# EnyaHermite/SPH3D-GCN

Measured on AMD Instinct MI355X. Metric: point-cloud blocks/sec (fwd+bwd) SPH3D_s3dis 8192-pt, higher is better.
Workload: dtype f32

## Files before the change

### sph3d_gcn_amd/csrc/conv3d.hip

```cpp
#include <stddef.h>
#include <string.h>
#include <type_traits>
#include "common.hpp"
#include "conv_plan.hpp"

namespace sph3d {

constexpr int kFwdSB = 4;
constexpr int kBatch = 8;

template <int R, int LPE, int SB>
__global__ __launch_bounds__(64 * kMultiWaves) void dwconv_fwd_multi(
    int B, int N, int M, int F, int C, int K, int mblocks, int nslices,
    const int* __restrict__ nnIndex, const int* __restrict__ nnCount, const int* __restrict__ binIndex,
    const float* __restrict__ input, const float* __restrict__ filter, float* __restrict__ output)
{
    extern __shared__ __attribute__((aligned(16))) float lfilt[];
    constexpr int EPL = 64 / LPE;
    constexpr int NO = 4 * R;
    constexpr int SLI = 4 * LPE;
    constexpr int FSTB = SLI * R * 4;
    const int CR = C * R;
    int b, part;
    xcd_decode((int)blockIdx.x, B, mblocks * nslices, b, part);
    if (b < 0) return;
    const int slice = part / mblocks;
    const int mb = part - slice * mblocks;
    const int ci0 = slice * SLI;
    const int SLi = (C - ci0) < SLI ? (C - ci0) : SLI;
    const int SLo = SLi * R;

    for (int e = threadIdx.x * 4; e < F * SLo; e += blockDim.x * 4) {
        const int f = e / SLo;
        const int cl = e - f * SLo;
        const int l4 = cl / (4 * R), q = (cl >> 2) % R;
        *reinterpret_cast<float4*>(&lfilt[f * (SLI * R) + q * SLI + l4 * 4]) =
            *reinterpret_cast<const float4*>(&filter[(size_t)f * CR + ci0 * R + cl]);
    }
    for (int e = threadIdx.x; e < SLI * R; e += blockDim.x) lfilt[F * (SLI * R) + e] = 0.f;
    __syncthreads();

    const int wave = uniform((int)threadIdx.x >> 6);
    const int lane = lane_id();
    const int g = lane / LPE;
    const int li = lane - g * LPE;
    const bool act = li * 4 < SLi;
    const int cic = act ? li * 4 : 0;
    const int m_begin = mb * kMultiPoints;
    const int m_end = (m_begin + kMultiPoints) < M ? (m_begin + kMultiPoints) : M;
    const char* inb = reinterpret_cast<const char*>(input + (size_t)b * N * C + ci0);
    const unsigned cicb = (unsigned)cic * 4u;
    const unsigned rowb = (unsigned)C * 4u;
    const char* lfb = reinterpret_cast<const char*>(lfilt);

    for (int m = m_begin + wave; m < m_end; m += kMultiWaves) {
        const size_t row = (size_t)b * M + m;
        const int cnt = uniform(nnCount[row]);
        float acc[NO];
#pragma unroll
        for (int v = 0; v < NO; v++) acc[v] = 0.f;
        for (int kt = 0; kt < cnt; kt += 64) {
            const int myk = kt + lane;
            const int kn = (cnt - kt) < 64 ? (cnt - kt) : 64;
            const int mykc = myk < cnt ? myk : kt;
            const int idxv = nnIndex[row * K + mykc];
            int binv = binIndex[row * K + mykc];
            binv = binv < 0 ? 0 : (binv >= F ? F - 1 : binv);
            binv = myk < cnt ? binv : F;
            const unsigned pk = ((unsigned)idxv & 0xffffffu) | ((unsigned)binv << 24);
            static_assert(64 % (SB * EPL) == 0, "batches must tile the 64-edge chunk (no index clamps)");
            for (int k0 = 0; k0 < kn; k0 += SB * EPL) {
                float4 x[SB];
                unsigned fo[SB];
#pragma unroll
                for (int u = 0; u < SB; u++) {
                    const int kq = k0 + u * EPL + g;
                    const unsigned p = (unsigned)__shfl((int)pk, kq);
                    const unsigned off = __umul24(p, rowb) + cicb;
                    fo[u] = __umul24(p >> 24, (unsigned)FSTB) + cicb;
                    x[u] = *reinterpret_cast<const float4*>(inb + off);
                }
#pragma unroll
                for (int u = 0; u < SB; u++) {
                    const float xs[4] = {x[u].x, x[u].y, x[u].z, x[u].w};
#pragma unroll
                    for (int q = 0; q < R; q++) {
                        const float4 w = *reinterpret_cast<const float4*>(lfb + fo[u] + q * (SLI * 4));
                        acc[4 * q + 0] = fmaf(xs[(4 * q + 0) / R], w.x, acc[4 * q + 0]);
                        acc[4 * q + 1] = fmaf(xs[(4 * q + 1) / R], w.y, acc[4 * q + 1]);
                        acc[4 * q + 2] = fmaf(xs[(4 * q + 2) / R], w.z, acc[4 * q + 2]);
                        acc[4 * q + 3] = fmaf(xs[(4 * q + 3) / R], w.w, acc[4 * q + 3]);
                    }
                }
            }
        }
#pragma unroll
        for (int o = LPE; o < 64; o <<= 1)
#pragma unroll
            for (int v = 0; v < NO; v++) acc[v] += __shfl_xor(acc[v], o);
        if (act && g == 0) {
            const float inv = cnt > 0 ? 1.0f / (float)cnt : 0.f;
            float* op = &output[row * CR + (size_t)(ci0 + li * 4) * R];
#pragma unroll
            for (int q = 0; q < R; q++) {
                float4 o;
                o.x = acc[4 * q + 0] * inv;
                o.y = acc[4 * q + 1] * inv;
                o.z = acc[4 * q + 2] * inv;
                o.w = acc[4 * q + 3] * inv;
                *reinterpret_cast<float4*>(&op[4 * q]) = o;
            }
        }
    }
}

template <int R>
__global__ __launch_bounds__(256) void dwconv_fwd_row(
    int B, int N, int M, int F, int C, int K, int mblocks, int nslices,
    const int* __restrict__ nnIndex, const int* __restrict__ nnCount, const int* __restrict__ binIndex,
    const float* __restrict__ input, const float* __restrict__ filter, float* __restrict__ output,
    const float* __restrict__ input2 = nullptr, int Ca = 0)
{
    extern __shared__ __attribute__((aligned(16))) float lfilt[];
    const int CR = C * R;
    int b, part;
    xcd_decode((int)blockIdx.x, B, mblocks * nslices, b, part);
    if (b < 0) return;
    const int slice = part / mblocks;
    const int mb = part - slice * mblocks;
    const int slice0 = slice * kSlice;
    const int SL = (CR - slice0) < kSlice ? (CR - slice0) : kSlice;

    for (int e = threadIdx.x * 4; e < F * SL; e += blockDim.x * 4) {
        const int f = e / SL;
        const int cl = e - f * SL;
        *reinterpret_cast<float4*>(&lfilt[e]) = *reinterpret_cast<const float4*>(&filter[(size_t)f * CR + slice0 + cl]);
    }
    for (int e = threadIdx.x; e < SL; e += blockDim.x) lfilt[F * SL + e] = 0.f;
    __syncthreads();

    const int wave = uniform((int)threadIdx.x >> 6);
    const int lane = lane_id();
    const int cl0 = lane * 4;
    const bool act = cl0 < SL;
    const int cin0 = (slice0 + cl0) / R;
    const int clc = act ? cl0 : 0;
    const int cinc = act ? cin0 : slice0 / R;
    const int m_begin = mb * kFwdPointsPerWG;
    const int m_end = (m_begin + kFwdPointsPerWG) < M ? (m_begin + kFwdPointsPerWG) : M;
    const bool second = input2 != nullptr && (slice0 / R) >= Ca;
    const int Cs = input2 == nullptr ? C : (second ? C - Ca : Ca);
    const int cshift = second ? Ca : 0;
    const float* inb = (second ? input2 : input) + (size_t)b * N * Cs - cshift;

    for (int m = m_begin + wave; m < m_end; m += 4) {
        const size_t row = (size_t)b * M + m;
        const int cnt = uniform(nnCount[row]);
        float4 acc = make_float4(0.f, 0.f, 0.f, 0.f);
        for (int kt = 0; kt < cnt; kt += 64) {
            const int myk = kt + lane;
            const int kn = (cnt - kt) < 64 ? (cnt - kt) : 64;
            const int mykc = myk < cnt ? myk : kt;
            const int idxv = nnIndex[row * K + mykc];
            int binv = binIndex[row * K + mykc];
            binv = binv < 0 ? 0 : (binv >= F ? F - 1 : binv);
            binv = myk < cnt ? binv : F;
            const unsigned noff = (unsigned)idxv * (unsigned)Cs;
            const int foff = binv * (SL >> 2);
            for (int k8 = 0; k8 < kn; k8 += kBatch) {
                unsigned n[kBatch];
                int f[kBatch];
#pragma unroll
                for (int u = 0; u < kBatch; u++) {
                    n[u] = (unsigned)__builtin_amdgcn_readlane((int)noff, k8 + u);
                    f[u] = __builtin_amdgcn_readlane(foff, k8 + u);
                }
                float4 w[kBatch];
                float4 x[kBatch];
#pragma unroll
                for (int u = 0; u < kBatch; u++) {
                    w[u] = reinterpret_cast<const float4*>(lfilt)[f[u] + (clc >> 2)];
                    const float* __restrict__ rp = inb + n[u];
                    if (R == 2) {
                        const float2 t = *reinterpret_cast<const float2*>(&rp[(unsigned)cinc]);
                        x[u] = make_float4(t.x, t.x, t.y, t.y);
                    } else {
                        x[u] = *reinterpret_cast<const float4*>(&rp[(unsigned)cinc]);
                    }
                }
#pragma unroll
                for (int u = 0; u < kBatch; u++) {
                    acc.x = fmaf(x[u].x, w[u].x, acc.x);
                    acc.y = fmaf(x[u].y, w[u].y, acc.y);
                    acc.z = fmaf(x[u].z, w[u].z, acc.z);
                    acc.w = fmaf(x[u].w, w[u].w, acc.w);
                }
            }
        }
        if (act) {
            const float inv = cnt > 0 ? 1.0f / (float)cnt : 0.f;
            float4 o;
            o.x = acc.x * inv;
            o.y = acc.y * inv;
            o.z = acc.z * inv;
            o.w = acc.w * inv;
            *reinterpret_cast<float4*>(&output[row * CR + slice0 + cl0]) = o;
        }
    }
}

__global__ __launch_bounds__(256) void dwconv_fwd_generic(
    int B, int N, int M, int F, int C, int r, int K, int mblocks, int nslices,
    const int* __restrict__ nnIndex, const int* __restrict__ nnCount, const int* __restrict__ binIndex,
    const float* __restrict__ input, const float* __restrict__ filter, float* __restrict__ output)
{
    extern __shared__ __attribute__((aligned(16))) float lfilt[];
    const int CR = C * r;
    int b, part;
    xcd_decode((int)blockIdx.x, B, mblocks * nslices, b, part);
    if (b < 0) return;
    const int slice = part / mblocks;
    const int mb = part - slice * mblocks;
    const int slice0 = slice * kSlice;
    const int SL = (CR - slice0) < kSlice ? (CR - slice0) : kSlice;

    for (int e = threadIdx.x; e < F * SL; e += blockDim.x) {
        const int f = e / SL;
        const int cl = e - f * SL;
        lfilt[e] = filter[(size_t)f * CR + slice0 + cl];
    }
    __syncthreads();

    const int wave = uniform((int)threadIdx.x >> 6);
    const int lane = lane_id();
    int cl[4], cin[4];
    bool act[4];
#pragma unroll
    for (int t = 0; t < 4; t++) {
        cl[t] = lane + 64 * t;
        act[t] = cl[t] < SL;
        cin[t] = act[t] ? (slice0 + cl[t]) / r : 0;
        if (!act[t]) cl[t] = 0;
    }
    const int m_begin = mb * kFwdPointsPerWG;
    const int m_end = (m_begin + kFwdPointsPerWG) < M ? (m_begin + kFwdPointsPerWG) : M;
    const float* inb = input + (size_t)b * N * C;

    for (int m = m_begin + wave; m < m_end; m += 4) {
        const size_t row = (size_t)b * M + m;
        const int cnt = uniform(nnCount[row]);
        float acc[4] = {0.f, 0.f, 0.f, 0.f};
        const int* __restrict__ irow = nnIndex + row * K;
        const int* __restrict__ brow = binIndex + row * K;
        {
#pragma unroll 4
            for (int kk = 0; kk < cnt; kk++) {
                const int n = irow[kk];
                int f = brow[kk];
                f = f < 0 ? 0 : (f >= F ? F - 1 : f);
#pragma unroll
                for (int t = 0; t < 4; t++) {
                    const float x = inb[(size_t)n * C + cin[t]];
                    const float w = lfilt[f * SL + cl[t]];
                    acc[t] = fmaf(x, w, acc[t]);
                }
            }
        }
#pragma unroll
        for (int t = 0; t < 4; t++) {
            if (act[t]) output[row * CR + slice0 + cl[t]] = cnt > 0 ? acc[t] / (float)cnt : 0.f;
        }
    }
}


constexpr int kBwdNL2 = 3;
constexpr int kBwdNL4 = 2;
template <int R, int V, int MAXF, int PARTS, bool COMPACT, int HUB = 0>
__global__ __launch_bounds__(kBwdTWaves * 64, COMPACT ? 4 : 3) void dwconv_bwd_t_vec(
    int B, int N, int M, int F, int C, int W, int parts, int nslices,
    const int* __restrict__ offsets, const int* __restrict__ entKey, const float* __restrict__ entScale,
    const int* __restrict__ order, const int* __restrict__ activeBins, int compactMax,
    const float* __restrict__ input, const float* __restrict__ filter, const float* __restrict__ gradOutput,
    float* __restrict__ gradInput, float* __restrict__ partial,
    const float* __restrict__ input2 = nullptr, float* __restrict__ gradInput2 = nullptr, int Ca = 0,
    int* __restrict__ hubList = nullptr, int hubT = 0, int slabBase = 0)
{
    extern __shared__ __attribute__((aligned(16))) float lds[];
    constexpr int SLW = 64 * V;
    constexpr int VI = (V >= R) ? V / R : 1;
    const int CR = C * R;
    const int A = activeBins ? uniform(activeBins[0]) : F;
    if (COMPACT ? (A > MAXF) : (activeBins != nullptr && A <= compactMax)) return;
    const int xcd = HUB == 2 ? 0 : ((int)blockIdx.x & 7);
    const int q = HUB == 2 ? (int)blockIdx.x : ((int)blockIdx.x >> 3);
    const int slice = q / W;
    const int w = q - slice * W;
    const int slice0 = slice * SLW;
    const int SL = (CR - slice0) < SLW ? (CR - slice0) : SLW;
    float* lfilt = lds;
    const bool second = input2 != nullptr && (slice0 / R) >= Ca;
    const int Cs = input2 == nullptr ? C : (second ? C - Ca : Ca);
    const float* __restrict__ xin = (second ? input2 : input) - (second ? Ca : 0);
    float* __restrict__ gin = (second ? gradInput2 : gradInput) - (second ? Ca : 0);

    for (int e = threadIdx.x * V; e < F * SL; e += blockDim.x * V) {
        const int f = e / SL;
        const int cl = e - f * SL;
#pragma unroll
        for (int v = 0; v < V; v++) lfilt[e + v] = filter[(size_t)f * CR + slice0 + cl + v];
    }
    __syncthreads();

    const int wave = uniform((int)threadIdx.x >> 6);
    const int lane = lane_id();
    const int stride = W * kBwdTWaves;
    constexpr bool HALF = PARTS > 1;
    constexpr int PL = 64 / PARTS;
    const int half = HALF ? (lane / PL) : 0;
    const int cl0 = (HALF ? (lane % PL) : lane) * V;
    const bool act = cl0 < SL;
    const int cin0 = (slice0 + cl0) / R;
    float acc[MAXF][V];
#pragma unroll
    for (int i = 0; i < MAXF; i++)
#pragma unroll
        for (int v = 0; v < V; v++) acc[i][v] = 0.f;

    const int abv = COMPACT ? activeBins[1 + ((lane < MAXF && lane < A) ? lane : 0)] : 0;

    const int nhub = HUB == 2 ? uniform(hubList[0]) : 0;
    for (int item = HUB == 2 ? w / kHubGroup : xcd; HUB == 2 ? item < nhub : item < B * parts; item += HUB == 2 ? W / kHubGroup : 8) {
    const int hubSrc = HUB == 2 ? uniform(hubList[1 + item]) : 0;
    const int b = HUB == 2 ? hubSrc / N : item / parts;
    const int pi = HUB == 2 ? 0 : item - b * parts;
    const float* __restrict__ gou = gradOutput + (size_t)b * M * CR + slice0;
    const unsigned cla = (unsigned)(act ? cl0 : 0);
    const int* __restrict__ offb = offsets + (size_t)b * ((size_t)N * F + 1);
    for (int p = HUB == 2 ? 0 : pi + parts * (w * kBwdTWaves + wave); HUB == 2 ? p < 1 : p < N; p += HUB == 2 ? 1 : parts * stride) {
        const int n = HUB == 2 ? hubSrc - b * N : (order ? uniform(order[(size_t)b * N + p]) : p);
        const int* __restrict__ o = offb + (size_t)n * F;
        const int ov0 = o[lane <= F ? lane : F];
        const int ov1 = (MAXF >= 64) ? o[(64 + lane) <= F ? (64 + lane) : F] : 0;
        float xi[VI], xv[V];
#pragma unroll
        for (int u = 0; u < VI; u++) xi[u] = xin[((size_t)b * N + n) * Cs + (act ? cin0 : slice0 / R) + u];
#pragma unroll
        for (int v = 0; v < V; v++) xv[v] = xi[(V >= R) ? v / R : 0];
        float gi[V];
#pragma unroll
        for (int v = 0; v < V; v++) gi[v] = 0.f;
        const int E0 = __builtin_amdgcn_readlane(ov0, 0);
        const int E1 = uniform(o[F]);
        unsigned long long nonempty = ~0ull;
        if (COMPACT) {
            const int fl = lane < MAXF ? abv : 0;
            const int s0 = __builtin_amdgcn_ds_bpermute(fl << 2, ov0);
            const int s1 = __builtin_amdgcn_ds_bpermute((fl + 1) << 2, ov0);
            nonempty = __ballot(s1 > s0);
        }
        if (HUB == 1 && (E1 - E0) > hubT) {
            if (slice == 0 && lane == 0) hubList[1 + atomicAdd(&hubList[0], 1)] = b * N + n;
            if (act && half == 0 && V >= R) {
                float* gp = &gin[((size_t)b * N + n) * Cs + cin0];
#pragma unroll
                for (int u = 0; u < VI; u++) gp[u] = 0.f;
            }
            continue;
        }
        const int cfirst = HUB == 2 ? E0 + 64 * ((w % kHubGroup) * kBwdTWaves + wave) : E0;
        const int cstep = HUB == 2 ? 64 * kHubGroup * kBwdTWaves : 64;
        for (int cb = cfirst; cb < E1; cb += cstep) {
        const int cn = (E1 - cb) < 64 ? (E1 - cb) : 64;
        const int li = lane < cn ? lane : 0;
        const int wkey = entKey[cb + li];
        const unsigned kel = (unsigned)tg_key(wkey, entScale == nullptr) * (unsigned)CR;
        const float svl = entScale == nullptr ? tg_packed_scale(wkey) : entScale[cb + li];
        const float sv = lane < cn ? svl : 0.f;
#pragma unroll
        for (int fi = 0; fi < MAXF; fi++) {
            if (fi < (COMPACT ? A : F) && (!COMPACT || ((nonempty >> (fi & 63)) & 1ull))) {
                const int f = COMPACT ? __builtin_amdgcn_readlane(abv, fi) : fi;
                const int a0 = COMPACT ? __builtin_amdgcn_readlane(ov0, f)
                                       : __builtin_amdgcn_readlane(fi < 64 ? ov0 : ov1, fi & 63);
                const int a1 = COMPACT ? __builtin_amdgcn_readlane(ov0, f + 1)
                                       : __builtin_amdgcn_readlane((fi + 1) < 64 ? ov0 : ov1, (fi + 1) & 63);
                const int e0 = (a0 > cb ? a0 : cb) - cb;
                const int e1 = (a1 < cb + cn ? a1 : cb + cn) - cb;
                if (e0 < e1) {
                    float sg[V];
#pragma unroll
                    for (int v = 0; v < V; v++) sg[v] = 0.f;
                    float wr[V];
                    {
                        const float* wrow = &lfilt[f * SL + (act ? cl0 : 0)];
#pragma unroll
                        for (int v = 0; v < V; v++) wr[v] = wrow[v];
                    }
                    if (HALF) {
                        constexpr int NL = PARTS == 2 ? kBwdNL2 : kBwdNL4;
                        const float svh = ((unsigned)(lane - e0) < (unsigned)(e1 - e0)) ? sv : 0.f;
#define SPH3D_BWD_HALF_BATCH(WRAPS)                                                                                  \
    {                                                                                                                \
        const int a4 = ((e + half) << 2);                                                                            \
        unsigned ko[NL];                                                                                             \
        float sc[NL];                                                                                                \
        _Pragma("unroll") for (int u = 0; u < NL; u++) {                                                             \
            ko[u] = (unsigned)__builtin_amdgcn_ds_bpermute(a4 + 4 * PARTS * u, (int)kel);                            \
            sc[u] = __int_as_float(__builtin_amdgcn_ds_bpermute(a4 + 4 * PARTS * u, __float_as_int(svh)));           \
            if (WRAPS) sc[u] = (e + half + PARTS * u) < 64 ? sc[u] : 0.f;                                            \
        }                                                                                                            \
        float g[NL][V];                                                                                              \
        _Pragma("unroll") for (int u = 0; u < NL; u++) {                                                             \
            const float4 t = *reinterpret_cast<const float4*>(&gou[ko[u] + cla]);                                    \
            g[u][0] = t.x; g[u][1 % V] = t.y; g[u][2 % V] = t.z; g[u][3 % V] = t.w;                                  \
        }                                                                                                            \
        _Pragma("unroll") for (int u = 0; u < NL; u++)                                                               \
            _Pragma("unroll") for (int v = 0; v < V; v++) sg[v] = fmaf(g[u][v], sc[u], sg[v]);                       \
    }
                        for (int e = e0; e < e1; e += PARTS * NL) {
                            if ((64 % (PARTS * NL)) != 0 && e + PARTS * NL > 64) SPH3D_BWD_HALF_BATCH(true)
                            else SPH3D_BWD_HALF_BATCH(false)
                        }
#undef SPH3D_BWD_HALF_BATCH
                    } else {
                    const float svm = ((unsigned)(lane - e0) < (unsigned)(e1 - e0)) ? sv : 0.f;
#define SPH3D_BWD_BATCH(NB)                                                                                          \
    {                                                                                                                \
        float sc[NB];                                                                                                \
        float g[NB][V];                                                                                              \
        _Pragma("unroll") for (int u = 0; u < NB; u++) {                                                             \
            const unsigned ko = (unsigned)__builtin_amdgcn_readlane((int)kel, e + u);                                \
            sc[u] = __int_as_float(__builtin_amdgcn_readlane(__float_as_int(svm), e + u));                           \
            const float* __restrict__ rp = gou + ko;                                   \
                        \
            if (V == 4) {                                                                                            \
                const float4 t = *reinterpret_cast<const float4*>(&rp[cla]);                                         \
                g[u][0] = t.x; g[u][1 % V] = t.y; g[u][2 % V] = t.z; g[u][3 % V] = t.w;                              \
            } else if (V == 2) {                                                                                     \
                const float2 t = *reinterpret_cast<const float2*>(&rp[cla]);                                         \
                g[u][0] = t.x; g[u][1 % V] = t.y;                                                                    \
            } else {                                                                                                 \
                g[u][0] = rp[cla];                                                                                   \
            }                                                                                                        \
        }                                                                                                            \
        _Pragma("unroll") for (int u = 0; u < NB; u++)                                                               \
            _Pragma("unroll") for (int v = 0; v < V; v++) sg[v] = fmaf(g[u][v], sc[u], sg[v]);                       \
    }
                    int e = e0;
                    for (; e + 4 <= e1; e += 4) SPH3D_BWD_BATCH(4)
                    const int rem = e1 - e;
                    if (rem == 3) SPH3D_BWD_BATCH(3)
                    else if (rem == 2) SPH3D_BWD_BATCH(2)
                    else if (rem == 1) SPH3D_BWD_BATCH(1)
#undef SPH3D_BWD_BATCH
                    }
#pragma unroll
                    for (int v = 0; v < V; v++) {
                        gi[v] = fmaf(sg[v], wr[v], gi[v]);
                        acc[fi][v] = fmaf(sg[v], xv[v], acc[fi][v]);
                    }
                }
            }
        }
        }
        if (HALF) {
#pragma unroll
            for (int v = 0; v < V; v++) {
                gi[v] += __shfl_xor(gi[v], 32);
                if (PARTS == 4) gi[v] += __shfl_xor(gi[v], 16);
            }
        }
        if (act && half == 0) {
            float* gp = &gin[((size_t)b * N + n) * Cs + cin0];
            if (V >= R) {
#pragma unroll
                for (int u = 0; u < VI; u++) {
                    float s = 0.f;
#pragma unroll
                    for (int rr = 0; rr < R; rr++) s += gi[u * R + rr];
                    if (HUB == 2) atomicAdd(&gp[u], s);
                    else gp[u] = s;
                }
            }
        }
    }

    }

    if (HALF) {
#pragma unroll
        for (int i = 0; i < MAXF; i++)
#pragma unroll
            for (int v = 0; v < V; v++) {
                acc[i][v] += __shfl_xor(acc[i][v], 32);
                if (PARTS == 4) acc[i][v] += __shfl_xor(acc[i][v], 16);
            }
    }
    __syncthreads();
    float* tab = lds;
    __shared__ unsigned long long activeMask;
    if (COMPACT) {
        if (threadIdx.x == 0) activeMask = 0ull;
        __syncthreads();
        if ((int)threadIdx.x < A) atomicOr(&activeMask, 1ull << activeBins[1 + threadIdx.x]);
        __syncthreads();
    }
    for (int w = 0; w < kBwdTWaves; w++) {
        if (wave == w && act && half == 0) {
#pragma unroll
            for (int i = 0; i < MAXF; i++) {
                if (i < (COMPACT ? A : F)) {
                    const int f = COMPACT ? uniform(activeBins[1 + i]) : i;
#pragma unroll
                    for (int v = 0; v < V; v++) {
                        float* p = &tab[f * SL + cl0 + v];
                        *p = (w == 0) ? acc[i][v] : (*p + acc[i][v]);
                    }
                }
            }
        }
        __syncthreads();
    }
    float* out = partial + (HUB == 2 ? (size_t)slabBase + w : (size_t)xcd * W + w) * ((size_t)F * CR);
    const unsigned long long am = COMPACT ? activeMask : ~0ull;
    for (int e = threadIdx.x; e < F * SL; e += blockDim.x) {
        const int f = e / SL;
        const int cl = e - f * SL;
        if (!COMPACT || ((am >> f) & 1ull)) out[(size_t)f * CR + slice0 + cl] = tab[e];
    }
}

__global__ __launch_bounds__(1024) void reduce_filter_partials(int nparts, int total, int CR, const float* __restrict__ partial,
                                                              float* __restrict__ gradFilter,
                                                              const int* __restrict__ activeBins, int compactMax, int npartsCompact)
{
    const bool compact = activeBins != nullptr && activeBins[0] <= compactMax;
    if (compact) nparts = npartsCompact;
    __shared__ float red[32][32];
    __shared__ unsigned long long activeMask;
    if (compact) {
        if (threadIdx.x == 0) activeMask = 0ull;
        __syncthreads();
        if ((int)threadIdx.x < activeBins[0]) atomicOr(&activeMask, 1ull << activeBins[1 + threadIdx.x]);
        __syncthreads();
    }
    const int cx = (int)threadIdx.x & 31, py = (int)threadIdx.x >> 5;
    const int j = blockIdx.x * 32 + cx;
    float s = 0.f;
    if (j < total && (!compact || ((activeMask >> (j / CR)) & 1ull))) {
        for (int p0 = py; p0 < nparts; p0 += 256) {
            float v[8];
#pragma unroll
            for (int u = 0; u < 8; u++) {
                const int p = p0 + u * 32;
                v[u] = partial[(size_t)(p < nparts ? p : py) * total + j];
            }
#pragma unroll
            for (int u = 0; u < 8; u++)
                if (p0 + u * 32 < nparts) s += v[u];
        }
    }
    red[py][cx] = s;
    __syncthreads();
    if (py == 0 && j < total) {
        for (int k = 1; k < 32; k++) s += red[k][cx];
        gradFilter[j] = s;
    }
}

__global__ __launch_bounds__(256) void dwconv_bwd_t_generic(
    int B, int N, int M, int F, int C, int r, int nblocks, int nslices, int sliceC,
    const int* __restrict__ offsets, const int* __restrict__ entKey, const float* __restrict__ entScale,
    const float* __restrict__ input, const float* __restrict__ filter, const float* __restrict__ gradOutput,
    float* __restrict__ gradInput, float* __restrict__ gradFilter)
{
    extern __shared__ __attribute__((aligned(16))) float gtab[];
    const int CR = C * r;
    int b, part;
    xcd_decode((int)blockIdx.x, B, nblocks * nslices, b, part);
    if (b < 0) return;
    const int slice = part / nblocks;
    const int nb = part - slice * nblocks;
    const int c_base = slice * sliceC;
    const int SC = (C - c_base) < sliceC ? (C - c_base) : sliceC;
    const int SW = SC * r;
    for (int e = threadIdx.x; e < F * SW; e += blockDim.x) gtab[e] = 0.f;
    __syncthreads();

    const int wave = uniform((int)threadIdx.x >> 6);
    const int lane = lane_id();
    const int n_begin = nb * 64;
    const int n_end = (n_begin + 64) < N ? (n_begin + 64) : N;
    const int* __restrict__ offb = offsets + (size_t)b * ((size_t)N * F + 1);
    for (int n = n_begin + wave; n < n_end; n += 4) {
        const int* __restrict__ o = offb + (size_t)n * F;
        for (int t = 0; t < 4; t++) {
            const int cl = lane + 64 * t;
            if (cl >= SC) break;
            const int cin = c_base + cl;
            const float x = input[((size_t)b * N + n) * C + cin];
            float gi = 0.f;
            for (int f = 0; f < F; f++) {
                const int e0 = o[f], e1 = o[f + 1];
                if (e0 >= e1) continue;
                for (int rr = 0; rr < r; rr++) {
                    const int cout = cin * r + rr;
                    float sg = 0.f;
                    for (int e = e0; e < e1; e++)
                        sg = fmaf(gradOutput[((size_t)b * M + tg_key(entKey[e], entScale == nullptr)) * CR + cout],
                                  entScale == nullptr ? tg_packed_scale(entKey[e]) : entScale[e], sg);
                    gi = fmaf(sg, filter[(size_t)f * CR + cout], gi);
                    unsafeAtomicAdd(&gtab[f * SW + cl * r + rr], sg * x);
                }
            }
            gradInput[((size_t)b * N + n) * C + cin] = gi;
        }
    }
    __syncthreads();
    for (int e = threadIdx.x; e < F * SW; e += blockDim.x) {
        const int f = e / SW;
        const int j = e - f * SW;
        const float g = gtab[e];
        if (g != 0.f) unsafeAtomicAdd(&gradFilter[(size_t)f * CR + c_base * r + j], g);
    }
}

template <int T, int MAXF>
__global__ __launch_bounds__(kBwdTWaves * 64, 3) void dwconv_bwd_t_odd(
    int B, int N, int M, int F, int C, int W, int parts, int nslices,
    const int* __restrict__ offsets, const int* __restrict__ entKey, const float* __restrict__ entScale,
    const int* __restrict__ order,
    const float* __restrict__ input, const float* __restrict__ filter, const float* __restrict__ gradOutput,
    float* __restrict__ gradInput, float* __restrict__ partial)
{
    extern __shared__ __attribute__((aligned(16))) float lds[];
    constexpr int SLW = 64 * T;
    const int xcd = (int)blockIdx.x & 7;
    const int q = (int)blockIdx.x >> 3;
    const int slice = q / W;
    const int w = q - slice * W;
    const int slice0 = slice * SLW;
    const int SL = (C - slice0) < SLW ? (C - slice0) : SLW;
    float* lfilt = lds;
    for (int e = threadIdx.x; e < F * SLW; e += blockDim.x) {
        const int f = e / SLW;
        const int cl = e - f * SLW;
        lfilt[e] = cl < SL ? filter[(size_t)f * C + slice0 + cl] : 0.f;
    }
    __syncthreads();

    const int wave = uniform((int)threadIdx.x >> 6);
    const int lane = lane_id();
    const int stride = W * kBwdTWaves;
    bool act[T];
    unsigned cla[T];
#pragma unroll
    for (int t = 0; t < T; t++) {
        act[t] = lane + 64 * t < SL;
        cla[t] = act[t] ? (unsigned)(lane + 64 * t) : 0u;
    }
    float acc[MAXF][T];
#pragma unroll
    for (int i = 0; i < MAXF; i++)
#pragma unroll
        for (int t = 0; t < T; t++) acc[i][t] = 0.f;

    for (int item = xcd; item < B * parts; item += 8) {
    const int b = item / parts;
    const int pi = item - b * parts;
    const float* __restrict__ gou = gradOutput + (size_t)b * M * C + slice0;
    const int* __restrict__ offb = offsets + (size_t)b * ((size_t)N * F + 1);
    for (int p = pi + parts * (w * kBwdTWaves + wave); p < N; p += parts * stride) {
        const int n = order ? uniform(order[(size_t)b * N + p]) : p;
        const int* __restrict__ o = offb + (size_t)n * F;
        const int ov0 = o[lane <= F ? lane : F];
        const int ov1 = (MAXF >= 64) ? o[(64 + lane) <= F ? (64 + lane) : F] : 0;
        const size_t xrow = ((size_t)b * N + n) * C + slice0;
        float xv[T], gi[T];
#pragma unroll
        for (int t = 0; t < T; t++) {
            xv[t] = input[xrow + cla[t]];
            gi[t] = 0.f;
        }
        const int E0 = __builtin_amdgcn_readlane(ov0, 0);
        const int E1 = uniform(o[F]);
        for (int cb = E0; cb < E1; cb += 64) {
        const int cn = (E1 - cb) < 64 ? (E1 - cb) : 64;
        const int li = lane < cn ? lane : 0;
        const int wkey = entKey[cb + li];
        const unsigned kel = (unsigned)tg_key(wkey, entScale == nullptr) * (unsigned)C;
        const float sv = entScale == nullptr ? tg_packed_scale(wkey) : entScale[cb + li];
#pragma unroll
        for (int fi = 0; fi < MAXF; fi++) {
            if (fi < F) {
                const int a0 = __builtin_amdgcn_readlane(fi < 64 ? ov0 : ov1, fi & 63);
                const int a1 = __builtin_amdgcn_readlane((fi + 1) < 64 ? ov0 : ov1, (fi + 1) & 63);
                const int e0 = (a0 > cb ? a0 : cb) - cb;
                const int e1 = (a1 < cb + cn ? a1 : cb + cn) - cb;
                if (e0 < e1) {
                    float sg[T], wr[T];
#pragma unroll
                    for (int t = 0; t < T; t++) {
                        sg[t] = 0.f;
                        wr[t] = lfilt[fi * SLW + 64 * t + lane];
                    }
#define SPH3D_BWD_ODD_BATCH(NB)                                                                                      \
    {                                                                                                                \
        float sc[NB];                                                                                                \
        float g[NB][T];                                                                                              \
        _Pragma("unroll") for (int u = 0; u < NB; u++) {                                                             \
            const unsigned ko = (unsigned)__builtin_amdgcn_readlane((int)kel, e + u);                                \
            sc[u] = __int_as_float(__builtin_amdgcn_readlane(__float_as_int(sv), e + u));                            \
            const float* __restrict__ rp = gou + ko;                                   \
            _Pragma("unroll") for (int t = 0; t < T; t++) g[u][t] = rp[cla[t]];                                      \
        }                                                                                                            \
        _Pragma("unroll") for (int u = 0; u < NB; u++)                                                               \
            _Pragma("unroll") for (int t = 0; t < T; t++) sg[t] = fmaf(g[u][t], sc[u], sg[t]);                       \
    }
                    int e = e0;
                    for (; e + 4 <= e1; e += 4) SPH3D_BWD_ODD_BATCH(4)
                    const int rem = e1 - e;
                    if (rem == 3) SPH3D_BWD_ODD_BATCH(3)
                    else if (rem == 2) SPH3D_BWD_ODD_BATCH(2)
                    else if (rem == 1) SPH3D_BWD_ODD_BATCH(1)
#undef SPH3D_BWD_ODD_BATCH
#pragma unroll
                    for (int t = 0; t < T; t++) {
                        gi[t] = fmaf(sg[t], wr[t], gi[t]);
                        acc[fi][t] = fmaf(sg[t], xv[t], acc[fi][t]);
                    }
                }
            }
        }
        }
#pragma unroll
        for (int t = 0; t < T; t++)
            if (act[t]) gradInput[xrow + cla[t]] = gi[t];
    }
    }

    __syncthreads();
    float* tab = lds;
    for (int tw = 0; tw < kBwdTWaves; tw++) {
        if (wave == tw) {
#pragma unroll
            for (int i = 0; i < MAXF; i++) {
                if (i < F) {
#pragma unroll
                    for (int t = 0; t < T; t++) {
                        float* p = &tab[i * SLW + 64 * t + lane];
                        *p = (tw == 0) ? acc[i][t] : (*p + acc[i][t]);
                    }
                }
            }
        }
        __syncthreads();
    }
    float* out = partial + ((size_t)xcd * W + w) * ((size_t)F * C);
    for (int e = threadIdx.x; e < F * SL; e += blockDim.x) {
        const int f = e / SL;
        const int cl = e - f * SL;
        out[(size_t)f * C + slice0 + cl] = tab[f * SLW + cl];
    }
}

}

using namespace sph3d;

struct ConvShape {
    int op, B, N, M, F, Ca, Cb, r, K;
};

static int hub_min_n() { return test_hook("SPH3D_BWD_HUB_MIN_N", 32768); }
static int hub_threshold() { const int t = test_hook("SPH3D_BWD_HUB_T", 1024); return t < 1 ? 1 : t; }

static ConvPlan plan_of(const ConvShape& s, bool active_given, bool deterministic = deterministic_on())
{
    const bool grad = s.op == kConvGradT || s.op == kConvGradTCat;
    return conv_plan(s.op, s.B, s.N, s.M, s.F, s.Ca, s.Cb, s.r, s.K, deterministic, active_given, grad ? hub_min_n() : 0,
                     grad ? hub_threshold() : 0);
}

static int plan_status(const ConvPlan& p, const ConvShape& s)
{
    const bool grad = s.op == kConvGradT || s.op == kConvGradTCat, cat = s.op == kConvFwdCat || s.op == kConvGradTCat;
    const char* who = grad ? "DepthwiseConv3dGrad" : "DepthwiseConv3d";
    const long long C = (long long)s.Ca + s.Cb;
    SPH3D_REQUIRE(p.bad != kConvBadDims, "%s: bad dims B=%d N=%d M=%d F=%d C=%lld r=%d K=%d", who, s.B, s.N, s.M, s.F, C, s.r, s.K);
    SPH3D_REQUIRE(p.bad != kConvBadLds, "%s: filter table slice F=%d does not fit LDS", who, s.F);
    SPH3D_REQUIRE(p.bad != kConvBadMultiplier, "%s: depth multiplier %d > 256 unsupported", who, s.r);
    SPH3D_REQUIRE(p.bad != kConvBadGrid, "%s: B=%d N=%d M=%d C=%lld r=%d is more than 2^31 - 1 workgroups", who, s.B, s.N, s.M, C, s.r);
    if (p.kernel != kConvRefused) return SPH3D_OK;
    if (cat)
        set_error("%s (two inputs): Ca=%d Cb=%d r=%d not covered (Ca*r must be a multiple of 256)", who, s.Ca, s.Cb, s.r);
    else
        set_error("DepthwiseConv3dGrad: deterministic mode is on and F=%d C=%lld r=%d takes the generic kernel, which sums with float "
                  "atomics (shapes with r in {1, 2} and F <= 65 run the fixed-order kernels)", s.F, C, s.r);
    return SPH3D_EUNSUPPORTED;
}

static int workspace_status(const void* workspace, size_t have, size_t need)
{
    if (need == 0 || (workspace != nullptr && have >= need)) return SPH3D_OK;
    set_error("DepthwiseConv3dGrad: workspace %zu B < required %zu B", have, need);
    return SPH3D_EWORKSPACE;
}

static int run_fwd(const ConvShape& s, const int* nn_index, const int* nn_count, const int* bin_index, const float* input,
                   const float* input2, const float* filter, float* output, sph3d_stream_t stream, const char* what)
{
    const ConvPlan p = plan_of(s, false);
    int rc = plan_status(p, s);
    if (rc || p.kernel == kConvNone) return rc;
    hipStream_t st = as_stream(stream);
    const int B = s.B, N = s.N, M = s.M, F = s.F, C = s.Ca + s.Cb, r = s.r, K = s.K, nslices = (int)p.nslices;
    static_assert(kMultiPoints == kFwdPointsPerWG, "one mblocks for the three kernels");
    const int mblocks = (int)((M + (long long)kFwdPointsPerWG - 1) / kFwdPointsPerWG);
    const dim3 grid((unsigned)p.grid);
    const size_t lds = (size_t)p.lds;
    if (p.kernel == kConvFwdMulti) {
        auto kern = p.LPE == 32 ? (p.R == 2 ? dwconv_fwd_multi<2, 32, kFwdSB> : dwconv_fwd_multi<1, 32, kFwdSB>)
                                : (p.R == 2 ? dwconv_fwd_multi<2, 16, kFwdSB> : dwconv_fwd_multi<1, 16, kFwdSB>);
        rc = launch_lds(kern, grid, dim3(64 * kMultiWaves), lds, st, "conv3d", B, N, M, F, C, K, mblocks, nslices, nn_index, nn_count,
                        bin_index, input, filter, output);
    } else if (p.kernel == kConvFwdRow) {
        rc = launch_lds(p.R == 2 ? dwconv_fwd_row<2> : dwconv_fwd_row<1>, grid, dim3(256), lds, st, "conv3d", B, N, M, F, C, K, mblocks,
                        nslices, nn_index, nn_count, bin_index, input, filter, output, input2, s.op == kConvFwdCat ? s.Ca : 0);
    } else {
        rc = launch_lds(dwconv_fwd_generic, grid, dim3(256), lds, st, "conv3d", B, N, M, F, C, r, K, mblocks, nslices, nn_index, nn_count,
                        bin_index, input, filter, output);
    }
    if (rc) return rc;
    return check_launch(what);
}

extern "C" int sph3d_depthwise_conv3d(int B, int N, int M, int F, int C, int r, int K,
                                      const int* nn_index, const int* nn_count, const int* bin_index,
                                      const float* input, const float* filter, float* output,
                                      sph3d_stream_t stream)
{
    return run_fwd({kConvFwd, B, N, M, F, C, 0, r, K}, nn_index, nn_count, bin_index, input, nullptr, filter, output, stream,
                   "sph3d_depthwise_conv3d");
}

extern "C" int sph3d_depthwise_conv3d_cat(int B, int N, int M, int F, int Ca, int Cb, int r, int K, const int* nn_index,
                                          const int* nn_count, const int* bin_index, const float* input_a, const float* input_b,
                                          const float* filter, float* output, sph3d_stream_t stream)
{
    return run_fwd({kConvFwdCat, B, N, M, F, Ca, Cb, r, K}, nn_index, nn_count, bin_index, input_a, input_b, filter, output, stream,
                   "sph3d_depthwise_conv3d_cat");
}

extern "C" int sph3d_depthwise_conv3d_cat_supported(int F, int Ca, int Cb, int r)
{
    return plan_of({kConvFwdCat, 1, 1, 1, F, Ca, Cb, r, 1}, false).kernel == kConvFwdRow;
}

struct GradArgs {
    const int *offsets, *ent_key;
    const float* ent_scale;
    const int *order, *active_bins;
    const float *input, *input2, *filter, *grad_output;
    float *grad_input, *grad_input2, *grad_filter;
    void* workspace;
};

template <int R, int V, int MAXF, int PARTS>
static int launch_bwd_t_vec(const ConvPlan& p, const ConvShape& s, const GradArgs& a, const int* ab, hipStream_t st)
{
    const int C = s.Ca + s.Cb, nslices = (int)p.nslices, T = (int)p.hub_threshold;
    int* hub_list = nullptr;
    if (p.hub) {
        hub_list = reinterpret_cast<int*>((char*)a.workspace + p.hub_list_offset);
        int rc = check_hip(hipMemsetAsync(hub_list, 0, sizeof(int), st), "conv3d grad: hub list");
        if (rc) return rc;
    }
    auto launch = [&](auto kern, long long wgs, long long W, long long parts, long long slab_base) {
        return launch_lds(kern, dim3((unsigned)(wgs * nslices)), dim3(kBwdTWaves * 64), (size_t)p.lds, st, "conv3d", s.B, s.N, s.M, s.F, C,
                          (int)W, (int)parts, nslices, a.offsets, a.ent_key, a.ent_scale, a.order, ab, kCompactBins, a.input, a.filter,
                          a.grad_output, a.grad_input, (float*)a.workspace, a.input2, a.grad_input2, s.op == kConvGradTCat ? s.Ca : 0,
                          hub_list, T, (int)slab_base);
    };
    auto sweep = [&](auto compact_table, const ConvTable& t) {
        constexpr bool CT = decltype(compact_table)::value;
        constexpr int MF = CT ? kCompactBins : MAXF;
        if constexpr (V == 4) {
            if (p.hub) {
                int rc = launch(dwconv_bwd_t_vec<R, V, MF, PARTS, CT, 1>, t.slabs, t.W, t.parts, 0);
                if (rc) return rc;
                return launch(dwconv_bwd_t_vec<R, V, MF, PARTS, CT, 2>, kHubWG, kHubWG, 1, t.slabs);
            }
        }
        return launch(dwconv_bwd_t_vec<R, V, MF, PARTS, CT, 0>, t.slabs, t.W, t.parts, 0);
    };
    if constexpr (V == 4) {
        if (p.compact_launch) {
            int rc = sweep(std::true_type{}, p.compact);
            if (rc) return rc;
        }
    }
    return sweep(std::false_type{}, p.full);
}

static int run_bwd_t_vec(const ConvPlan& p, const ConvShape& s, const GradArgs& a, const int* ab, hipStream_t st)
{
    using std::integral_constant;
    auto go = [&](auto R, auto V, auto PARTS) { return launch_bwd_t_vec<R(), V(), (V() == 4 ? 33 : 65), PARTS()>(p, s, a, ab, st); };
    auto with_r = [&](auto R) {
        if (p.V == 2) return go(R, integral_constant<int, 2>{}, integral_constant<int, 1>{});
        if (p.PARTS == 4) return go(R, integral_constant<int, 4>{}, integral_constant<int, 4>{});
        if (p.PARTS == 2) return go(R, integral_constant<int, 4>{}, integral_constant<int, 2>{});
        return go(R, integral_constant<int, 4>{}, integral_constant<int, 1>{});
    };
    return p.R == 2 ? with_r(integral_constant<int, 2>{}) : with_r(integral_constant<int, 1>{});
}

static int run_bwd_t_odd(const ConvPlan& p, const ConvShape& s, const GradArgs& a, hipStream_t st)
{
    auto go = [&](auto kern) {
        return launch_lds(kern, dim3((unsigned)p.grid), dim3(kBwdTWaves * 64), (size_t)p.lds, st, "conv3d", s.B, s.N, s.M, s.F, s.Ca,
                          (int)p.full.W, (int)p.full.parts, (int)p.nslices, a.offsets, a.ent_key, a.ent_scale, a.order, a.input, a.filter,
                          a.grad_output, a.grad_input, (float*)a.workspace);
    };
    const int T = (int)p.V;
    if (p.MAXF == 33) return T == 1 ? go(dwconv_bwd_t_odd<1, 33>) : T == 2 ? go(dwconv_bwd_t_odd<2, 33>)
                           : T == 3 ? go(dwconv_bwd_t_odd<3, 33>) : go(dwconv_bwd_t_odd<4, 33>);
    return T == 1 ? go(dwconv_bwd_t_odd<1, 65>) : go(dwconv_bwd_t_odd<2, 65>);
}

static int run_grad_t(const ConvShape& s, const GradArgs& a, size_t workspace_bytes, sph3d_stream_t stream)
{
    const ConvPlan p = plan_of(s, a.active_bins != nullptr);
    int rc = plan_status(p, s);
    if (rc) return rc;
    hipStream_t st = as_stream(stream);
    const int C = s.Ca + s.Cb, CR = C * s.r, total = s.F * CR;
    if (p.kernel == kConvNone || p.kernel == kConvBwdGeneric) {
        rc = check_hip(hipMemsetAsync(a.grad_filter, 0, sizeof(float) * (size_t)total, st), "conv3d grad: memset");
        if (rc || p.kernel == kConvNone) return rc;
    }
    rc = workspace_status(a.workspace, workspace_bytes, (size_t)p.workspace_bytes);
    if (rc) return rc;
    const int* ab = p.compact_launch ? a.active_bins : nullptr;
    if (p.kernel == kConvBwdVec) {
        rc = run_bwd_t_vec(p, s, a, ab, st);
    } else if (p.kernel == kConvBwdOdd) {
        rc = run_bwd_t_odd(p, s, a, st);
    } else {
        const int sliceC = (int)(p.lds / ((long long)sizeof(float) * s.F * s.r));
        rc = launch_lds(dwconv_bwd_t_generic, dim3((unsigned)p.grid), dim3(256), (size_t)p.lds, st, "conv3d", s.B, s.N, s.M, s.F, C, s.r,
                        (int)((s.N + 63LL) / 64), (int)p.nslices, sliceC, a.offsets, a.ent_key, a.ent_scale, a.input, a.filter,
                        a.grad_output, a.grad_input, a.grad_filter);
    }
    if (rc) return rc;
    if (p.reduce_slabs)
        hipLaunchKernelGGL(reduce_filter_partials, dim3((total + 31) / 32), dim3(1024), 0, st, (int)p.reduce_slabs, total, CR,
                           (const float*)a.workspace, a.grad_filter, ab, p.kernel == kConvBwdVec ? kCompactBins : 0,
                           (int)p.reduce_slabs_compact);
    return check_launch("sph3d_depthwise_conv3d_grad_t");
}

extern "C" int sph3d_depthwise_conv3d_grad_t(int B, int N, int M, int F, int C, int r,
                                             const int* offsets, const int* ent_key, const float* ent_scale,
                                             const int* source_order, const int* active_bins,
                                             const float* input, const float* filter, const float* grad_output,
                                             float* grad_input, float* grad_filter,
                                             void* workspace, size_t workspace_bytes, sph3d_stream_t stream)
{
    return run_grad_t({kConvGradT, B, N, M, F, C, 0, r, 1}, {offsets, ent_key, ent_scale, source_order, active_bins, input, nullptr, filter,
                      grad_output, grad_input, nullptr, grad_filter, workspace}, workspace_bytes, stream);
}

extern "C" int sph3d_depthwise_conv3d_grad_t_cat(int B, int N, int M, int F, int Ca, int Cb, int r, const int* offsets, const int* ent_key,
                                                 const float* ent_scale, const int* source_order, const int* active_bins,
                                                 const float* input_a, const float* input_b, const float* filter,
                                                 const float* grad_output, float* grad_a, float* grad_b, float* grad_filter,
                                                 void* workspace, size_t workspace_bytes, sph3d_stream_t stream)
{
    return run_grad_t({kConvGradTCat, B, N, M, F, Ca, Cb, r, 1}, {offsets, ent_key, ent_scale, source_order, active_bins, input_a, input_b,
                      filter, grad_output, grad_a, grad_b, grad_filter, workspace}, workspace_bytes, stream);
}

extern "C" size_t sph3d_depthwise_conv3d_grad_t_workspace(int B, int N, int F, int C, int r)
{
    return (size_t)plan_of({kConvGradT, B, N, 0, F, C, 0, r, 1}, false).workspace_bytes;
}
extern "C" size_t sph3d_depthwise_conv3d_grad_workspace(int B, int N, int M, int F, int C, int r, int K)
{
    return tg_layout(nullptr, B, N, M, K, F).bytes + sph3d_depthwise_conv3d_grad_t_workspace(B, N, F, C, r);
}

extern "C" int sph3d_depthwise_conv3d_grad(int B, int N, int M, int F, int C, int r, int K,
                                           const int* nn_index, const int* nn_count, const int* bin_index,
                                           const float* input, const float* filter, const float* grad_output,
                                           float* grad_input, float* grad_filter,
                                           void* workspace, size_t workspace_bytes, sph3d_stream_t stream)
{
    const ConvShape with_k = {kConvGradT, B, N, M, F, C, 0, r, K}, s = {kConvGradT, B, N, M, F, C, 0, r, 1};
    int rc = plan_status(plan_of(with_k, true), with_k);
    if (rc) return rc;
    GradArgs a = {nullptr, nullptr, nullptr, nullptr, nullptr, input, nullptr, filter, grad_output, grad_input, nullptr, grad_filter, nullptr};
    if (B == 0) return run_grad_t(s, a, 0, stream);
    const TgLayout t = tg_layout(workspace, B, N, M, K, F);
    rc = workspace_status(workspace, workspace_bytes, sph3d_depthwise_conv3d_grad_workspace(B, N, M, F, C, r, K));
    if (rc) return rc;
    rc = sph3d_graph_transpose(B, N, M, K, F, nn_index, nn_count, bin_index, nullptr, t.offsets, t.key, t.scale, t.active,
                               t.scratch, t.scratch_bytes, stream);
    if (rc) return rc;
    a.offsets = t.offsets, a.ent_key = t.key, a.ent_scale = t.scale, a.active_bins = t.active, a.workspace = (char*)workspace + t.bytes;
    return run_grad_t(s, a, workspace_bytes - t.bytes, stream);
}

extern "C" int sph3d_depthwise_conv3d_plan(int op, int B, int N, int M, int F, int Ca, int Cb, int r, int K, int deterministic,
                                           int active_given, long long* out)
{
    const bool grad = op == kConvGradT || op == kConvGradTCat, cat = op == kConvFwdCat || op == kConvGradTCat;
    SPH3D_REQUIRE(out != nullptr && op >= kConvFwd && op <= kConvGradTCat && deterministic >= -1 && deterministic <= 1 &&
                      (active_given == 0 || active_given == 1) && (cat || Cb == 0),
                  "sph3d_depthwise_conv3d_plan: bad argument (op=%d deterministic=%d active_given=%d Cb=%d out=%p)", op, deterministic,
                  active_given, Cb, (void*)out);
    const ConvShape s = {op, B, N, M, F, Ca, Cb, r, grad ? 1 : K};
    const ConvPlan p = plan_of(s, active_given != 0, deterministic < 0 ? deterministic_on() : deterministic != 0);
    if (p.bad) return plan_status(p, s);
    static_assert(offsetof(ConvPlan, bad) == SPH3D_CONV_PLAN_FIELDS * sizeof(long long), "the plan starts with the documented fields, in their order");
    static_assert(kConvFwd == SPH3D_CONV_FWD && kConvFwdCat == SPH3D_CONV_FWD_CAT && kConvGradT == SPH3D_CONV_GRAD_T && kConvGradTCat == SPH3D_CONV_GRAD_T_CAT,
                  "the ops as the header numbers them");
    memcpy(out, &p, SPH3D_CONV_PLAN_FIELDS * sizeof(long long));
    return SPH3D_OK;
}
```

Baseline: 2098.

## Software-pipeline point metadata and first key chunk loads in backward depthwise conv

Restructures the per-point loop of the backward depthwise conv kernel so the next point's source index, offset bounds, edge range and first chunk of entry keys are loaded one iteration ahead, with indices prefetched up to three points out. This is meant to hide global-memory latency on the dependent order→offsets→entKey load chain. It also folds the active-bin check into the ballot mask and uses an asm barrier to force per-lane offset addressing. The cost is higher register pressure and extra loads at the tail, where indices are clamped to N-1.

```diff
diff --git a/sph3d_gcn_amd/csrc/conv3d.hip b/sph3d_gcn_amd/csrc/conv3d.hip
--- a/sph3d_gcn_amd/csrc/conv3d.hip
+++ b/sph3d_gcn_amd/csrc/conv3d.hip
@@ -337,27 +337,69 @@
     const float* __restrict__ gou = gradOutput + (size_t)b * M * CR + slice0;
     const unsigned cla = (unsigned)(act ? cl0 : 0);
     const int* __restrict__ offb = offsets + (size_t)b * ((size_t)N * F + 1);
-    for (int p = HUB == 2 ? 0 : pi + parts * (w * kBwdTWaves + wave); HUB == 2 ? p < 1 : p < N; p += HUB == 2 ? 1 : parts * stride) {
-        const int n = HUB == 2 ? hubSrc - b * N : (order ? uniform(order[(size_t)b * N + p]) : p);
-        const int* __restrict__ o = offb + (size_t)n * F;
-        const int ov0 = o[lane <= F ? lane : F];
-        const int ov1 = (MAXF >= 64) ? o[(64 + lane) <= F ? (64 + lane) : F] : 0;
+    const int pstep = HUB == 2 ? 1 : parts * stride;
+    const int pfirst = HUB == 2 ? 0 : pi + parts * (w * kBwdTWaves + wave);
+    if (HUB != 2 && pfirst >= N) continue;
+    auto src_at = [&](int q) {
+        const int qc = q < N ? q : N - 1;
+        return order ? uniform(order[(size_t)b * N + qc]) : qc;
+    };
+    auto lane_offset = [](int i) {
+        unsigned u = (unsigned)i;
+        asm volatile("" : "+v"(u));
+        return u;
+    };
+    auto bounds0 = [&](int nn) { return (offb + (size_t)nn * F)[lane_offset(lane <= F ? lane : F)]; };
+    auto bounds1 = [&](int nn) { return (MAXF >= 64) ? (offb + (size_t)nn * F)[lane_offset((64 + lane) <= F ? (64 + lane) : F)] : 0; };
+    auto keys0 = [&](int e0, int e1) {
+        const int c = (e1 - e0) < 64 ? (e1 - e0) : 64;
+        return e1 > e0 ? (entKey + e0)[(unsigned)(lane < c ? lane : 0)] : 0;
+    };
+    int n1 = 0, n2 = 0, n3 = 0, E0n = 0, E1n = 0, E0nn = 0, E1nn = 0, ovn0 = 0, ovn1 = 0, wkn = 0;
+    if (HUB != 2) {
+        n1 = src_at(pfirst);
+        n2 = src_at(pfirst + pstep);
+        n3 = src_at(pfirst + 2 * pstep);
+        E0n = uniform(offb[(size_t)n1 * F]);
+        E1n = uniform(offb[(size_t)n1 * F + F]);
+        E0nn = uniform(offb[(size_t)n2 * F]);
+        E1nn = uniform(offb[(size_t)n2 * F + F]);
+        ovn0 = bounds0(n1);
+        ovn1 = bounds1(n1);
+        wkn = keys0(E0n, E1n);
+    }
+    for (int p = pfirst; HUB == 2 ? p < 1 : p < N; p += pstep) {
+        int n, ov0, ov1, E0, E1, wkey0 = 0;
+        if (HUB == 2) {
+            n = hubSrc - b * N;
+            ov0 = bounds0(n);
+            ov1 = bounds1(n);
+            E0 = __builtin_amdgcn_readlane(ov0, 0);
+            E1 = uniform(offb[(size_t)n * F + F]);
+        } else {
+            n = n1, ov0 = ovn0, ov1 = ovn1, E0 = E0n, E1 = E1n, wkey0 = wkn;
+            n1 = n2, n2 = n3, E0n = E0nn, E1n = E1nn;
+            n3 = src_at(p + 3 * pstep);
+            E0nn = uniform(offb[(size_t)n2 * F]);
+            E1nn = uniform(offb[(size_t)n2 * F + F]);
+            ovn0 = bounds0(n1);
+            ovn1 = bounds1(n1);
+            wkn = keys0(E0n, E1n);
+        }
         float xi[VI], xv[V];
 #pragma unroll
-        for (int u = 0; u < VI; u++) xi[u] = xin[((size_t)b * N + n) * Cs + (act ? cin0 : slice0 / R) + u];
+        for (int u = 0; u < VI; u++) xi[u] = (xin + ((size_t)b * N + n) * Cs)[lane_offset(act ? cin0 : slice0 / R) + u];
 #pragma unroll
         for (int v = 0; v < V; v++) xv[v] = xi[(V >= R) ? v / R : 0];
         float gi[V];
 #pragma unroll
         for (int v = 0; v < V; v++) gi[v] = 0.f;
-        const int E0 = __builtin_amdgcn_readlane(ov0, 0);
-        const int E1 = uniform(o[F]);
         unsigned long long nonempty = ~0ull;
         if (COMPACT) {
             const int fl = lane < MAXF ? abv : 0;
             const int s0 = __builtin_amdgcn_ds_bpermute(fl << 2, ov0);
             const int s1 = __builtin_amdgcn_ds_bpermute((fl + 1) << 2, ov0);
-            nonempty = __ballot(s1 > s0);
+            nonempty = __ballot(s1 > s0 && lane < A);
         }
         if (HUB == 1 && (E1 - E0) > hubT) {
             if (slice == 0 && lane == 0) hubList[1 + atomicAdd(&hubList[0], 1)] = b * N + n;
@@ -370,16 +412,22 @@
         }
         const int cfirst = HUB == 2 ? E0 + 64 * ((w % kHubGroup) * kBwdTWaves + wave) : E0;
         const int cstep = HUB == 2 ? 64 * kHubGroup * kBwdTWaves : 64;
-        for (int cb = cfirst; cb < E1; cb += cstep) {
-        const int cn = (E1 - cb) < 64 ? (E1 - cb) : 64;
-        const int li = lane < cn ? lane : 0;
-        const int wkey = entKey[cb + li];
-        const unsigned kel = (unsigned)tg_key(wkey, entScale == nullptr) * (unsigned)CR;
-        const float svl = entScale == nullptr ? tg_packed_scale(wkey) : entScale[cb + li];
-        const float sv = lane < cn ? svl : 0.f;
+        int cb = cfirst, cn = 0;
+        unsigned kel = 0u;
+        float sv = 0.f;
+        auto take_chunk = [&](bool prefetched) {
+            cn = (E1 - cb) < 64 ? (E1 - cb) : 64;
+            const int li = lane < cn ? lane : 0;
+            const int wkey = prefetched ? wkey0 : (entKey + cb)[(unsigned)li];
+            kel = (unsigned)tg_key(wkey, entScale == nullptr) * (unsigned)CR;
+            const float svl = entScale == nullptr ? tg_packed_scale(wkey) : (entScale + cb)[(unsigned)li];
+            sv = lane < cn ? svl : 0.f;
+        };
+        if (cb < E1) take_chunk(HUB != 2);
+        while (cb < E1) {
 #pragma unroll
         for (int fi = 0; fi < MAXF; fi++) {
-            if (fi < (COMPACT ? A : F) && (!COMPACT || ((nonempty >> (fi & 63)) & 1ull))) {
+            if (COMPACT ? ((nonempty >> (fi & 63)) & 1ull) != 0ull : fi < F) {
                 const int f = COMPACT ? __builtin_amdgcn_readlane(abv, fi) : fi;
                 const int a0 = COMPACT ? __builtin_amdgcn_readlane(ov0, f)
                                        : __builtin_amdgcn_readlane(fi < 64 ? ov0 : ov1, fi & 63);
@@ -463,6 +511,8 @@
                 }
             }
         }
+        cb += cstep;
+        if (cb < E1) take_chunk(false);
         }
         if (HALF) {
 #pragma unroll
@@ -472,7 +522,7 @@
             }
         }
         if (act && half == 0) {
-            float* gp = &gin[((size_t)b * N + n) * Cs + cin0];
+            float* gp = &(gin + ((size_t)b * N + n) * Cs)[lane_offset(cin0)];
             if (V >= R) {
 #pragma unroll
                 for (int u = 0; u < VI; u++) {
```

New measurement: 2128 (median of 6 runs). 1.4% higher.
